# jonassibbesen/rpvg

Measured on AMD Instinct MI355X. Metric: read-pairs quantified/sec, higher is better.
Workload: dtype f64

## Files before the change

### include/rpvg_hip.h

```cpp
#ifndef RPVG_HIP_H
#define RPVG_HIP_H

#include <stdint.h>

#include "rpvg_batch.h"
#include "rpvg_rows.h"
#include "rpvg_index.h"
#include "rpvg_table.h"

#ifdef __cplusplus
extern "C" {
#endif

typedef enum rpvg_hip_status {
    RPVG_HIP_OK = 0,
    RPVG_HIP_ERR_NO_DEVICE = -1,
    RPVG_HIP_ERR_RUNTIME = -2,
    RPVG_HIP_ERR_INVALID = -3,
    RPVG_HIP_ERR_ALLOC = -4,
    RPVG_HIP_ERR_UNSUPPORTED = -5
} rpvg_hip_status;

typedef struct rpvg_hip_ctx rpvg_hip_ctx;
typedef struct rpvg_hip_batch rpvg_hip_batch;
// ... 71 lines not shown
                                double * device_matrix, uint64_t ld, double * device_counts, double * total_count);

typedef struct rpvg_hip_group_spec {
    uint32_t num_matrices;
    const uint32_t * cluster;
    const uint64_t * group_off;
    const uint64_t * group_path_off;
    const uint32_t * group_path;
    int32_t normalise;
    double collapse_precision;
} rpvg_hip_group_spec;

int rpvg_hip_groups_build(rpvg_hip_ctx * ctx, const rpvg_hip_batch * batch, const rpvg_hip_group_spec * spec,
                          rpvg_hip_groups ** groups_out);
int rpvg_hip_groups_build_from_sources(rpvg_hip_ctx * ctx, const rpvg_hip_batch * batch, uint32_t num_matrices,
                                       const uint32_t * clusters, int32_t normalise, double collapse_precision,
                                       rpvg_hip_groups ** groups_out);
int rpvg_hip_groups_build_single_paths(rpvg_hip_ctx * ctx, const rpvg_hip_batch * batch, uint32_t num_matrices,
                                       const uint32_t * clusters, int32_t normalise, double collapse_precision,
                                       rpvg_hip_groups ** groups_out);
void rpvg_hip_groups_free(rpvg_hip_ctx * ctx, rpvg_hip_groups * groups);
int rpvg_hip_groups_collapse_info(rpvg_hip_ctx * ctx, const rpvg_hip_groups * groups, uint32_t * matrices_replayed,
                                  uint32_t * rows_replaced, uint32_t * matrices_sorted_whole, uint32_t * active_rows);

int rpvg_hip_group_loglik(rpvg_hip_ctx * ctx, const rpvg_hip_groups * groups, uint32_t num_requests,
                          const uint32_t * matrix, const uint32_t * members, uint32_t width, double divisor,
                          const uint8_t * add_rowmax, double * out);

int rpvg_hip_group_conditionals(rpvg_hip_ctx * ctx, const rpvg_hip_groups * groups, uint32_t num_requests,
                                const uint32_t * matrix, const uint32_t * others, uint32_t width, double divisor,
                                double * out);

#define RPVG_HIP_FULL_MAX_SETS 0x7fffffffull
int rpvg_hip_group_full_posteriors(rpvg_hip_ctx * ctx, const rpvg_hip_groups * groups, uint32_t num_problems,
                                   const uint32_t * matrix, uint32_t group_size, const double * log_freq,
                                   double * posteriors);
uint64_t rpvg_hip_full_set_count(uint32_t columns, uint32_t group_size);

typedef struct rpvg_hip_gibbs_spec {
    uint32_t num_problems;
    uint32_t group_size;
    const uint32_t * matrix;
    const uint32_t * num_chains;
    const uint32_t * num_burn_its;
    const uint32_t * num_gibbs_its;
    const double * log_freq;
// ... 205 lines not shown
```

### rpvg_amd/csrc/row_collapse.hip

```cpp

#include "common.hpp"

#include <hipcub/hipcub.hpp>

#include <cfloat>

using namespace rpvg_hip_detail;

namespace {

constexpr int kKeyFractionBits = kCollapseKeyFractionBits;
constexpr uint32_t kMaxWindowCompares = 256;
enum : uint8_t { kRowListed = 1, kRowStoodFor = 2 };
constexpr int kCsrCellHashBits = 8;
constexpr double kEquivalentRelative = 1e-13;
constexpr uint32_t kListLdsRows = 2048;
constexpr uint32_t kSortThreads = 256;
constexpr uint32_t kBetweenThreads = 256;
constexpr uint32_t kBetweenRows = 2 * kBetweenThreads;
constexpr uint32_t kPairChunk = 256;
constexpr uint32_t kWholeMatrixBit = 0x80000000u;
constexpr uint32_t kBigListBit = 0x40000000u;
constexpr uint32_t kListSizeMask = 0x3FFFFFFFu;
constexpr uint32_t kPairwiseRows = 1024;
// ... 1134 lines not shown
        if (a.rewritten_count[m] == 0) continue;
        __syncthreads();
        adjustSearchSums(a, m, item % kAdjustSlices);
    }
}

__global__ __launch_bounds__(256) void collapseRewriteKernel(const ReplayArgs<MatrixArrays> a) {
    __shared__ uint32_t demote;
    const uint32_t num_items = a.replay_list[a.num_matrices];
    for (uint32_t item = blockIdx.x; item < num_items; item += gridDim.x) {
        const uint32_t m = a.replay_list[item];
        const uint32_t encoded = a.mat_list[m];
        __syncthreads();
        if (threadIdx.x == 0) demote = 0;
        __syncthreads();
        finishRuns(a, m, encoded & kListSizeMask, a.order + 2 * a.g.rowOffset(m), a.head_of + a.g.rowOffset(m), &demote, (encoded & kWholeMatrixBit) != 0);
    }
}

}

namespace {

constexpr uint32_t kSmallSortRows = 1024;
constexpr uint32_t kSmallSortThreads = 128;
constexpr uint32_t kSortChunkRows = 2048;
constexpr uint32_t kSortChunkThreads = 256;
constexpr uint32_t kMergeTile = 1024;
constexpr uint32_t kMergeThreads = 128;
constexpr uint32_t kSortRowBits = 20;
constexpr uint64_t kSortMaxSegmentRows = (1ull << kSortRowBits) - 1;

template <int HASH>
__device__ __forceinline__ uint64_t packSortWord(const uint64_t key, const uint32_t row) {
    constexpr int low = kCollapseLargestBits - HASH;
    const uint64_t sorted = (key & ((1ull << kCollapseMatrixShift) - 1)) >> low;
    return (sorted << (kSortRowBits + low)) | (static_cast<uint64_t>(row) << low) | (key & ((1ull << low) - 1));
}
template <int HASH>
__device__ __forceinline__ uint32_t sortWordRow(const uint64_t word) { return static_cast<uint32_t>(word >> (kCollapseLargestBits - HASH)) & ((1u << kSortRowBits) - 1); }
template <int HASH>
__device__ __forceinline__ uint64_t sortWordKey(const uint64_t word, const uint32_t matrix) {
    constexpr int low = kCollapseLargestBits - HASH;
    return (static_cast<uint64_t>(matrix) << kCollapseMatrixShift) | ((word >> (kSortRowBits + low)) << low) | (word & ((1ull << low) - 1));
}
template <int HASH>
__device__ __forceinline__ bool sortWordsSameSortedPart(const uint64_t x, const uint64_t y) {
    constexpr int shift = kSortRowBits + kCollapseLargestBits - HASH;
    return HASH ? (x >> shift) == (y >> shift) : ((x >> shift) == (y >> shift) && ((x ^ y) & ((1ull << (kCollapseLargestBits - HASH)) - 1)) == 0);
}

__device__ __forceinline__ uint64_t cellHashTerm(const uint32_t column, const double value) {
    const uint64_t cell = static_cast<uint64_t>(cellOf(value));
// ... 8 lines not shown
    return key_in[r0 + i];
}
__device__ __forceinline__ uint64_t sortKeyOfRow(const CsrArrays & g, const uint32_t p, const uint64_t r0, const uint32_t i, const uint64_t * key_in,
                                                 uint64_t * pattern_out) {
    (void) key_in;
    const CsrView mv = g.view(p);
    const double noise = mv.noise[i];
    double projection = collapseWeight(mv.G) * noise, largest = 0.0;
    uint64_t cells = cellHashTerm(mv.G, noise), pattern = 0;
    for (uint32_t e = mv.off[i]; e < mv.off[i + 1]; ++e) {
        const uint32_t c = mv.col[e];
        const double v = mv.val[e];
        projection = fma(collapseWeight(c), v, projection);
        largest = fmax(largest, v);
        cells += cellHashTerm(c, v);
        if (c < 64 && v != 0.0) pattern |= 1ull << c;
    }
    pattern_out[r0 + i] = pattern;
    constexpr int low_bits = kCollapseLargestBits - kCsrCellHashBits;
    uint64_t k = collapseSortKey(p, projection, largest);
    k = (k & ~((1ull << kCollapseLargestBits) - 1)) | (((cells * 0x9E3779B97F4A7C15ull) >> (64 - kCsrCellHashBits)) << low_bits) | (k & ((1ull << low_bits) - 1));
    return k;
}

template <typename Arrays>
struct SegmentSortArgs {
    Arrays g;
    uint32_t num_matrices;
    const uint32_t * num_matrices_dev;
    uint32_t num_items_bound;
    const uint32_t * num_items_dev;
    const uint64_t * seg_first;
    const uint32_t * item_problem;
    uint32_t segment_rows;
    uint64_t total_rows;
    const uint64_t * key_in;
    uint64_t * pattern_out;
    uint64_t * sort_key;
    uint32_t * sort_row;
    uint32_t * position_of;
    uint8_t * same_prev;
    uint32_t * stretch_start;
    uint64_t * words_a, * words_b;
    uint32_t * chunks;
    uint32_t * chunk_count;
    uint32_t chunk_capacity;
    uint32_t round;
    uint32_t rounds;
};

template <typename Arrays>
__device__ __forceinline__ void writeSortedPosition(const SegmentSortArgs<Arrays> & a, const uint32_t m, const uint64_t r0, const uint64_t position, const uint64_t word,
                                                    const uint64_t word_before, const bool has_before) {
    constexpr int HASH = Arrays::kHashBits;
    const uint32_t row = sortWordRow<HASH>(word);
    uint8_t same = 0;
    if (has_before && sortWordsSameSortedPart<HASH>(word, word_before)) {
        const typename Arrays::View mv = viewOf(m, a.g);
        const uint32_t before = sortWordRow<HASH>(word_before);
        same = (HASH ? rowsSameCells(mv, row, before) : rowsIdentical(mv, row, before)) ? 1 : 0;
    }
    a.sort_key[position] = sortWordKey<HASH>(word, m);
    a.sort_row[position] = static_cast<uint32_t>(r0 + row);
    a.position_of[r0 + row] = static_cast<uint32_t>(position);
    a.same_prev[position] = same;
    a.stretch_start[position] = same ? 0u : static_cast<uint32_t>(position);
}

template <typename Arrays>
__device__ __forceinline__ void sortChunkInLds(const SegmentSortArgs<Arrays> & a, const uint32_t m, const uint64_t r0, const uint64_t c0, const uint32_t n,
                                               const uint32_t padded, uint64_t * words) {
    constexpr int HASH = Arrays::kHashBits;
    for (uint32_t i = threadIdx.x; i < padded; i += blockDim.x) {
        words[i] = i < n ? packSortWord<HASH>(sortKeyOfRow(a.g, m, r0, static_cast<uint32_t>(c0 + i), a.key_in, a.pattern_out), static_cast<uint32_t>(c0 + i)) : ~0ull;
    }
    __syncthreads();
    for (uint32_t k = 2; k <= padded; k <<= 1) {
        for (uint32_t j = k >> 1; j > 0; j >>= 1) {
            for (uint32_t t = threadIdx.x; t < (padded >> 1); t += blockDim.x) {
                const uint32_t i = ((t & ~(j - 1)) << 1) | (t & (j - 1));
                const uint32_t l = i | j;
                const uint64_t x = words[i], y = words[l];
                if (((i & k) == 0) == (x > y)) {
                    words[i] = y;
                    words[l] = x;
                }
            }
            __syncthreads();
        }
    }
}

template <typename Arrays>
__global__ __launch_bounds__(kSmallSortThreads) void collapseSmallSortKernel(const SegmentSortArgs<Arrays> a) {
    __shared__ uint64_t words[kSmallSortRows];
    const uint32_t M = a.num_matrices_dev ? min(*a.num_matrices_dev, a.num_matrices) : a.num_matrices;
    for (uint32_t m = blockIdx.x; m < M; m += gridDim.x) {
        const uint64_t R = a.g.numRows(m);
        if (R == 0) continue;
        if (R > kSmallSortRows) {
            if (threadIdx.x == 0) {
                const uint32_t chunks = static_cast<uint32_t>((R + kSortChunkRows - 1) / kSortChunkRows);
                const uint32_t first = atomicAdd(a.chunk_count, chunks);
                for (uint32_t c = 0; c < chunks && first + c < a.chunk_capacity; ++c) {
                    a.chunks[2 * static_cast<uint64_t>(first + c)] = m;
                    a.chunks[2 * static_cast<uint64_t>(first + c) + 1] = c;
                }
            }
            continue;
        }
        const uint64_t r0 = a.g.rowOffset(m);
        const uint32_t n = static_cast<uint32_t>(R);
        uint32_t padded = 2;
        while (padded < n) padded <<= 1;
        __syncthreads();
        sortChunkInLds(a, m, r0, 0, n, padded, words);
        for (uint32_t i = threadIdx.x; i < n; i += blockDim.x) writeSortedPosition(a, m, r0, r0 + i, words[i], i ? words[i - 1] : 0ull, i != 0);
    }
}

template <typename Arrays>
__global__ __launch_bounds__(kSortChunkThreads) void collapseChunkSortKernel(const SegmentSortArgs<Arrays> a) {
    __shared__ uint64_t words[kSortChunkRows];
    const uint32_t count = min(*a.chunk_count, a.chunk_capacity);
    for (uint32_t item = blockIdx.x; item < count; item += gridDim.x) {
        const uint32_t m = a.chunks[2 * static_cast<uint64_t>(item)], chunk = a.chunks[2 * static_cast<uint64_t>(item) + 1];
        const uint64_t R = a.g.numRows(m), r0 = a.g.rowOffset(m);
        const uint64_t c0 = static_cast<uint64_t>(chunk) * kSortChunkRows;
        const uint32_t n = static_cast<uint32_t>(min(static_cast<uint64_t>(kSortChunkRows), R - c0));
        uint32_t padded = 64;
        while (padded < n) padded <<= 1;
        __syncthreads();
        sortChunkInLds(a, m, r0, c0, n, padded, words);
        for (uint32_t i = threadIdx.x; i < n; i += blockDim.x) a.words_a[r0 + c0 + i] = words[i];
    }
}

template <typename Arrays>
__global__ __launch_bounds__(kMergeThreads) void collapseMergeRoundKernel(const SegmentSortArgs<Arrays> a) {
    constexpr uint32_t kPerThread = kMergeTile / kMergeThreads;
    constexpr uint32_t kTilesPerChunk = kSortChunkRows / kMergeTile;
    const uint32_t count = min(*a.chunk_count, a.chunk_capacity) * kTilesPerChunk;
    const uint64_t * __restrict__ source = (a.round & 1) ? a.words_b : a.words_a;
    uint64_t * __restrict__ target = (a.round & 1) ? a.words_a : a.words_b;
    const uint64_t run = static_cast<uint64_t>(kSortChunkRows) << a.round;
    for (uint32_t item = blockIdx.x; item < count; item += gridDim.x) {
        const uint32_t m = a.chunks[2 * static_cast<uint64_t>(item / kTilesPerChunk)];
        const uint64_t R = a.g.numRows(m), r0 = a.g.rowOffset(m);
        const uint64_t out0 = static_cast<uint64_t>(a.chunks[2 * static_cast<uint64_t>(item / kTilesPerChunk) + 1]) * kSortChunkRows + (item % kTilesPerChunk) * kMergeTile;
        if (out0 >= R) continue;
        const uint64_t pair0 = out0 / (2 * run) * (2 * run);
        const uint64_t a1 = min(R, pair0 + run), b1 = min(R, pair0 + 2 * run);
        const uint64_t * A = source + r0 + pair0, * B = source + r0 + a1;
        const uint64_t nA = a1 - pair0, nB = b1 - a1;
        const uint64_t d = (out0 - pair0) + static_cast<uint64_t>(threadIdx.x) * kPerThread;
        if (d >= nA + nB) continue;
        uint64_t lo = d > nB ? d - nB : 0, hi = min(d, nA);
        while (lo < hi) {
            const uint64_t mid = (lo + hi) >> 1;
            if (A[mid] < B[d - mid - 1]) lo = mid + 1;
            else hi = mid;
        }
        uint64_t i = lo, j = d - lo;
        uint64_t * out = target + r0 + pair0 + d;
        const uint32_t outputs = static_cast<uint32_t>(min(static_cast<uint64_t>(kPerThread), nA + nB - d));
        uint64_t x = i < nA ? A[i] : ~0ull, y = j < nB ? B[j] : ~0ull;
        for (uint32_t k = 0; k < outputs; ++k) {
            if (x < y) {
                out[k] = x;
                ++i;
                x = i < nA ? A[i] : ~0ull;
            } else {
                out[k] = y;
                ++j;
                y = j < nB ? B[j] : ~0ull;
            }
        }
    }
}

template <typename Arrays>
__global__ __launch_bounds__(256) void collapseMergedPositionsKernel(const SegmentSortArgs<Arrays> a) {
    const uint32_t count = min(*a.chunk_count, a.chunk_capacity);
    const uint64_t * __restrict__ sorted = (a.rounds & 1) ? a.words_b : a.words_a;
    for (uint32_t item = blockIdx.x; item < count; item += gridDim.x) {
        const uint32_t m = a.chunks[2 * static_cast<uint64_t>(item)], chunk = a.chunks[2 * static_cast<uint64_t>(item) + 1];
        const uint64_t R = a.g.numRows(m), r0 = a.g.rowOffset(m);
        const uint64_t c0 = static_cast<uint64_t>(chunk) * kSortChunkRows;
        const uint32_t n = static_cast<uint32_t>(min(static_cast<uint64_t>(kSortChunkRows), R - c0));
        for (uint32_t e = threadIdx.x; e < n; e += blockDim.x) {
            const uint64_t i = c0 + e;
            writeSortedPosition(a, m, r0, r0 + i, sorted[r0 + i], i ? sorted[r0 + i - 1] : 0ull, i != 0);
        }
    }
}

template <typename Arrays>
__global__ __launch_bounds__(256) void collapseUnusedSlotsKernel(const SegmentSortArgs<Arrays> a) {
    const uint32_t M = a.num_matrices_dev ? min(*a.num_matrices_dev, a.num_matrices) : a.num_matrices;
    const uint32_t items = a.num_items_dev ? min(*a.num_items_dev, a.num_items_bound) : a.num_items_bound;
    const uint64_t unused = collapseSortKey(a.num_matrices, 0.0, 0.0);
    auto fill = [&](const uint64_t r) {
        a.sort_key[r] = unused;
        a.sort_row[r] = static_cast<uint32_t>(r);
        a.position_of[r] = static_cast<uint32_t>(r);
        a.same_prev[r] = 0;
        a.stretch_start[r] = static_cast<uint32_t>(r);
        a.pattern_out[r] = 0;
    };
    for (uint32_t item = blockIdx.x; item < items; item += gridDim.x) {
// ... 36 lines not shown
    DeviceBuffer<uint32_t> row_out, order, head, pair_column, marked_list, pairs, between_items, row_items, list_index;
    DeviceBuffer<uint32_t> stretch;
    DeviceBuffer<uint64_t> pair_base;
    DeviceBuffer<uint8_t> pair_table;
    DeviceBuffer<double> pair_bound;
    DeviceBuffer<uint8_t> bytes;
    DeviceBuffer<unsigned char> sort_tmp;
    DeviceBuffer<uint64_t> csr_key, csr_pattern;
    DeviceBuffer<uint32_t> csr_row, csr_segments;
    DeviceBuffer<uint64_t> words_a, words_b;
    DeviceBuffer<uint32_t> chunks, chunk_count;
};

struct SegmentSortPlan {
    const uint32_t * num_matrices_dev = nullptr;
    uint32_t num_items_bound = 0;
    const uint32_t * num_items_dev = nullptr;
    const uint64_t * seg_first = nullptr;
    const uint32_t * item_problem = nullptr;
    uint32_t segment_rows = 0;
    uint64_t * pattern_out = nullptr;
    uint64_t max_segment_rows = 0;
};

template <typename Arrays>
hipError_t queueCollapseStages(const Arrays & arrays, const uint32_t M, const uint64_t total_rows, const double precision, const uint64_t * key,
                               const uint32_t * row, const uint32_t * segment_begin, const uint32_t * segment_end, const bool segmented, DeviceBuffer<uint32_t> & info, double * rowmax, uint32_t * mat_fast,
                               uint32_t * mat_mid, CollapseTemporaries * tmp, hipStream_t st, const SegmentSortPlan * plan = nullptr, hipEvent_t sorted = nullptr,
                               std::function<hipError_t(hipStream_t, const SearchParts *)> * held_back_runs = nullptr) {
    hipError_t e = hipSuccess;
    auto ok = [&](hipError_t r) { if (e == hipSuccess) e = r; return e == hipSuccess; };
    const uint64_t mark_words = (total_rows + 31) / 32;
    const uint64_t num_words = 2 + 2 * static_cast<uint64_t>(M) + 1 + mark_words + 5;
    const uint32_t pair_capacity = static_cast<uint32_t>(std::min<uint64_t>(4 * total_rows + 4096, 0x20000000ull));
    if (tmp->key_out.count != total_rows) ok(tmp->key_out.alloc(total_rows));
    if (tmp->row_out.count != total_rows) ok(tmp->row_out.alloc(total_rows));
    const uint64_t active_words = (total_rows + 3) / 4;
    ok(info.alloc(kInfoWords + num_words + active_words + M));
    ok(tmp->order.alloc(2 * total_rows));
    ok(tmp->head.alloc(total_rows));
    ok(tmp->pair_column.alloc(total_rows));
    ok(tmp->pair_bound.alloc(2 * total_rows));
    ok(tmp->pair_pattern.alloc(total_rows));
    ok(tmp->marked_list.alloc(total_rows));
    ok(tmp->pairs.alloc(2 * static_cast<size_t>(pair_capacity)));
    ok(tmp->between_items.alloc(2 * (total_rows / kBetweenRows + M)));
// ... 3 lines not shown
    ok(tmp->pair_table.alloc(kPairTableBytes));
    ok(tmp->bytes.alloc(3 * total_rows));
    ok(tmp->stretch.alloc(4 * total_rows));
    int matrix_bits = 1;
    while ((1u << matrix_bits) < M + 1) ++matrix_bits;
    const int begin_bit = kCollapseLargestBits - Arrays::kHashBits, end_bit = segmented ? kCollapseMatrixShift : kCollapseMatrixShift + matrix_bits;
    size_t sort_bytes = 0;
    auto sort = [&](void * scratch) {
        return segmented ? hipcub::DeviceSegmentedRadixSort::SortPairs(scratch, sort_bytes, key, tmp->key_out.ptr, row,
                                                                       tmp->row_out.ptr, static_cast<int>(total_rows), static_cast<int>(M),
                                                                       segment_begin, segment_end, begin_bit, end_bit, st)
                         : hipcub::DeviceRadixSort::SortPairs(scratch, sort_bytes, key, tmp->key_out.ptr, row,
                                                              tmp->row_out.ptr, static_cast<int>(total_rows), begin_bit, end_bit, st);
    };
    if (e == hipSuccess && !plan) ok(sort(nullptr));
    uint32_t * stretch_start = tmp->stretch.ptr, * stretch_first = stretch_start + total_rows, * stretch_end = stretch_first + total_rows,
             * position_of = stretch_end + total_rows;
    size_t scan_bytes = 0;
    auto scan = [&](void * scratch) {
        return hipcub::DeviceScan::InclusiveScan(scratch, scan_bytes, stretch_start, stretch_first, hipcub::Max(), static_cast<int>(total_rows), st);
    };
    if (e == hipSuccess) ok(scan(nullptr));
    ok(tmp->sort_tmp.alloc(std::max(sort_bytes, scan_bytes)));
    uint32_t chunk_capacity = 0, merge_rounds = 0;
    if (plan) {
        chunk_capacity = static_cast<uint32_t>(std::min<uint64_t>(total_rows / kSortChunkRows + M + 1, 0x7fffffffull));
        const uint64_t max_chunks = (plan->max_segment_rows + kSortChunkRows - 1) / kSortChunkRows;
        while ((1ull << merge_rounds) < max_chunks) ++merge_rounds;
        ok(tmp->words_a.alloc(total_rows));
        ok(tmp->words_b.alloc(total_rows));
        ok(tmp->chunks.alloc(2 * static_cast<size_t>(chunk_capacity)));
        ok(tmp->chunk_count.alloc(1));
    }
    if (e != hipSuccess) return e;
    uint32_t * pair_bytes = info.ptr + kInfoWords, * mat_flag = pair_bytes + 2, * replay_list = mat_flag + M, * marked_bits = replay_list + M + 1,
             * marked_count = marked_bits + mark_words, * pair_counts = marked_count + 1, * between_count = pair_counts + 2,
             * row_item_count = between_count + 1, * mat_list = pair_bytes + num_words + active_words;
    uint8_t * same_prev = tmp->bytes.ptr, * close = same_prev + total_rows, * barrier = close + total_rows;
    uint8_t * active = reinterpret_cast<uint8_t *>(pair_bytes + num_words);
    ok(zeroAsync(info.ptr, (kInfoWords + num_words + active_words) * sizeof(uint32_t), st));
    if (!plan) ok(sort(tmp->sort_tmp.ptr));
    PairScanArgs<Arrays> a;
    a.total_rows = total_rows;
    a.precision = precision;
    a.sort_key = tmp->key_out.ptr;
    a.sort_row = tmp->row_out.ptr;
    a.g = arrays;
    a.same_prev = same_prev;
    a.stretch_first = stretch_start;
    a.stretch_end = stretch_end;
    a.position_of = position_of;
// ... 15 lines not shown
        SegmentSortArgs<Arrays> c;
        c.g = arrays;
        c.num_matrices = M;
        c.num_matrices_dev = plan->num_matrices_dev;
        c.num_items_bound = plan->num_items_bound;
        c.num_items_dev = plan->num_items_dev;
        c.seg_first = plan->seg_first;
        c.item_problem = plan->item_problem;
        c.segment_rows = plan->segment_rows;
        c.total_rows = total_rows;
        c.key_in = key;
        c.pattern_out = plan->pattern_out;
        c.sort_key = tmp->key_out.ptr;
        c.sort_row = tmp->row_out.ptr;
        c.position_of = position_of;
        c.same_prev = same_prev;
        c.stretch_start = stretch_start;
        c.words_a = tmp->words_a.ptr;
        c.words_b = tmp->words_b.ptr;
        c.chunks = tmp->chunks.ptr;
        c.chunk_count = tmp->chunk_count.ptr;
        c.chunk_capacity = chunk_capacity;
        c.round = 0;
        c.rounds = merge_rounds;
        if (Arrays::kHashBits) {
            collapseUnusedSlotsKernel<Arrays><<<dim3(std::max<uint32_t>(1, std::min<uint32_t>(plan->num_items_bound, 8 * small_grid))), dim3(256), 0, st>>>(c);
        }
        collapseSmallSortKernel<Arrays><<<dim3(std::max<uint32_t>(1, std::min<uint32_t>(M, 16 * small_grid))), dim3(kSmallSortThreads), 0, st>>>(c);
        if (plan->max_segment_rows > kSmallSortRows) {
            collapseChunkSortKernel<Arrays><<<dim3(4 * small_grid), dim3(kSortChunkThreads), 0, st>>>(c);
            for (uint32_t round = 0; round < merge_rounds; ++round) {
                c.round = round;
                collapseMergeRoundKernel<Arrays><<<dim3(8 * small_grid), dim3(kMergeThreads), 0, st>>>(c);
            }
            collapseMergedPositionsKernel<Arrays><<<dim3(4 * small_grid), dim3(256), 0, st>>>(c);
        }
    } else {
        collapseSamePrevKernel<Arrays><<<dim3(row_blocks), dim3(256), 0, st>>>(a);
    }
    if (sorted) ok(hipEventRecord(sorted, st));
    ok(scan(tmp->sort_tmp.ptr));
    a.stretch_first = stretch_first;
    collapseStretchEndKernel<Arrays><<<dim3(row_blocks), dim3(256), 0, st>>>(a);
    collapseForwardPairsKernel<Arrays><<<dim3(row_blocks), dim3(256), 0, st>>>(a);
    collapseMarkPairsKernel<Arrays><<<dim3(small_grid), dim3(64), 0, st>>>(a);
    a.pair_count = pair_counts + 1;
    collapseAroundPairsKernel<Arrays><<<dim3(256), dim3(64), 0, st>>>(a);
    collapseActivePairsKernel<Arrays><<<dim3(small_grid), dim3(64), 0, st>>>(a);
    ReplayArgs<Arrays> r;
    r.num_matrices = M;
    r.precision = precision;
    r.g = arrays;
    r.mat_flag = mat_flag;
    r.active = active;
    r.sort_row = tmp->row_out.ptr;
    r.position_of = position_of;
    r.stretch_end = stretch_end;
    r.rowmax = rowmax;
    r.mat_fast = mat_fast;
// ... 205 lines not shown
    ok(hipGetLastError());
    if (e != hipSuccess) return e;
    return queueCollapseStages(arrays, P, total_rows, precision, tmp->csr_key.ptr, tmp->csr_row.ptr, segment_begin, segment_end, segmented, work.info, nullptr,
                               nullptr, nullptr, tmp.get(), st, nullptr, sorted);
}

extern "C" int rpvg_hip_groups_collapse_info(rpvg_hip_ctx * ctx, const rpvg_hip_groups * groups, uint32_t * matrices_replayed,
                                             uint32_t * rows_replaced, uint32_t * matrices_sorted_whole, uint32_t * active_rows) {
    RPVG_REQUIRE(ctx && groups, "rpvg_hip_groups_collapse_info: NULL argument");
    uint32_t info[kInfoWords] = {0};
    if (groups->collapse_info.ptr) {
        std::lock_guard<std::mutex> lock(ctx->mutex);
        RPVG_HIP_CHECK(hipSetDevice(ctx->device));
        RPVG_HIP_CHECK(groups->waitCollapse(ctx->stream));
        RPVG_HIP_CHECK(hipMemcpyAsync(info, groups->collapse_info.ptr, sizeof(info), hipMemcpyDeviceToHost, ctx->stream));
        RPVG_HIP_CHECK(hipStreamSynchronize(ctx->stream));
    }
    if (matrices_replayed) *matrices_replayed = info[kInfoMatrices];
    if (rows_replaced) *rows_replaced = info[kInfoRowsReplaced];
    if (matrices_sorted_whole) *matrices_sorted_whole = info[kInfoWholeMatrices];
    if (active_rows) *active_rows = info[kInfoActiveRows];
    return RPVG_HIP_OK;
}
```

### rpvg_amd/hip.py

```python
from __future__ import annotations

import ctypes as C
import os
from typing import List, Optional, Sequence, Tuple

import numpy as np

from .batch import CClusterBatch, ClusterBatch

_HERE = os.path.dirname(os.path.abspath(__file__))
LIB_PATH = os.path.join(_HERE, "csrc", "librpvg_hip.so")

EXPORTS = [
    "rpvg_hip_device_count", "rpvg_hip_create", "rpvg_hip_create_uploader", "rpvg_hip_destroy", "rpvg_hip_last_error", "rpvg_hip_synchronize",
    "rpvg_hip_device_info", "rpvg_hip_malloc", "rpvg_hip_free", "rpvg_hip_memcpy_h2d", "rpvg_hip_memcpy_d2h",
    "rpvg_hip_batch_upload", "rpvg_hip_batch_free", "rpvg_hip_em_solve", "rpvg_hip_em_dense",
    "rpvg_hip_dense_from_cluster", "rpvg_hip_groups_build", "rpvg_hip_groups_free", "rpvg_hip_groups_collapse_info", "rpvg_hip_group_loglik",
    "rpvg_hip_synth_dense_cluster", "rpvg_hip_stats_get", "rpvg_hip_stats_reset", "rpvg_hip_stats_intervals", "rpvg_hip_em_kernel_name",
    "rpvg_hip_gibbs_read_counts", "rpvg_hip_min_path_cover", "rpvg_hip_min_path_cover_any", "rpvg_hip_cover_limits", "rpvg_hip_bounded_pair_posteriors", "rpvg_hip_pair_posteriors_get", "rpvg_hip_pair_posteriors_free",
    "rpvg_hip_em_dense_sharded", "rpvg_hip_synth_dense_rows", "rpvg_hip_synth_dense_cluster_batch", "rpvg_hip_comm_unique_id", "rpvg_hip_comm_init",
    "rpvg_hip_comm_destroy", "rpvg_hip_comm_allreduce_sum_f64", "rpvg_hip_comm_init_all", "rpvg_hip_gather", "rpvg_hip_host_register", "rpvg_hip_host_unregister", "rpvg_hip_group_conditionals",
    "rpvg_hip_group_gibbs", "rpvg_hip_group_gibbs_polyploid", "rpvg_hip_gibbs_sets_get", "rpvg_hip_gibbs_sets_free",
    "rpvg_hip_alignments_upload", "rpvg_hip_alignments_free", "rpvg_hip_read_rows_build", "rpvg_hip_read_rows_to_batch",
    "rpvg_hip_read_rows_view", "rpvg_hip_read_rows_sizes", "rpvg_hip_read_rows_free", "rpvg_hip_path_clusters", "rpvg_hip_debug_log",
    "rpvg_hip_nested_subset_em", "rpvg_hip_subset_em_get", "rpvg_hip_subset_em_free",
    "rpvg_hip_batch_cluster_totals", "rpvg_hip_batch_has_source_columns", "rpvg_hip_batch_source_columns_sizes",
    "rpvg_hip_batch_source_columns_get", "rpvg_hip_groups_build_from_sources", "rpvg_hip_groups_build_single_paths", "rpvg_hip_batch_upload_begin", "rpvg_hip_batch_upload_finish", "rpvg_hip_create_with_streams",
    "rpvg_hip_batch_upload_finish_queue", "rpvg_hip_batch_upload_finish_wait",
    "rpvg_hip_batch_upload_segments", "rpvg_hip_pinned_alloc", "rpvg_hip_pinned_free", "rpvg_hip_thread_wait_spin_us",
    "rpvg_hip_group_full_posteriors", "rpvg_hip_full_set_count",
    "rpvg_hip_frag_length_fit", "rpvg_hip_frag_length_table", "rpvg_hip_frag_length_table_get", "rpvg_hip_frag_length_table_free",
    "rpvg_hip_effective_lengths", "rpvg_hip_alignments_set_effective_lengths", "rpvg_hip_frag_length_eval",
    "rpvg_hip_align_index_create", "rpvg_hip_align_index_free", "rpvg_hip_align_index_add", "rpvg_hip_align_index_finish",
    "rpvg_hip_align_index_frag_counts", "rpvg_hip_align_index_view", "rpvg_hip_align_index_alignments",
    "rpvg_hip_path_table_upload", "rpvg_hip_path_table_free", "rpvg_hip_read_rows_to_batch_with_paths", "rpvg_hip_batch_path_group_ids",
    "rpvg_hip_name_groups_limits", "rpvg_hip_align_index_name_groups", "rpvg_hip_name_groups_view", "rpvg_hip_name_groups_free",
    "rpvg_hip_estimates_table_build", "rpvg_hip_estimates_table_tpm", "rpvg_hip_estimates_table_view", "rpvg_hip_estimates_table_limits",
    "rpvg_hip_estimates_table_free",
    "rpvg_hip_align_index_alignments_collapsed",
    "rpvg_hip_batch_rows_sizes", "rpvg_hip_batch_rows_get",
]

COMM_ID_BYTES = 128


class EngineError(RuntimeError):
    pass


class CEmProblems(C.Structure):
    _fields_ = [("num_problems", C.c_uint32), ("cluster", C.c_void_p), ("col_off", C.c_void_p), ("col_path", C.c_void_p),
                ("collapse_precision", C.c_double)]


class CEmResults(C.Structure):
    _fields_ = [("abundances", C.c_void_p), ("noise_count", C.c_void_p), ("total_count", C.c_void_p),
                ("iterations", C.c_void_p)]


class CGroupSpec(C.Structure):
    _fields_ = [("num_matrices", C.c_uint32), ("cluster", C.c_void_p), ("group_off", C.c_void_p),
                ("group_path_off", C.c_void_p), ("group_path", C.c_void_p), ("normalise", C.c_int32),
                ("collapse_precision", C.c_double)]
# ... 625 lines not shown
        _check(lib().rpvg_hip_gibbs_read_counts(self.handle, batch.handle, C.byref(probs), C.c_void_p(init.ctypes.data),
                                                C.c_void_p(init_noise.ctypes.data), C.c_void_p(n.ctypes.data), C.c_void_p(sd.ctypes.data),
                                                C.c_uint32(thin), C.c_double(gamma), C.c_void_p(noise.ctypes.data),
                                                C.c_void_p(abund.ctypes.data)), "rpvg_hip_gibbs_read_counts")
        out, at_n, at_a = [], 0, 0
        for p in range(P):
            k, w = int(n[p]), int(widths[p])
            out.append((noise[at_n:at_n + k], abund[at_a:at_a + k * w].reshape(k, w)))
            at_n, at_a = at_n + k, at_a + k * w
        return out

    def min_path_cover(self, batch: DeviceBatch, clusters: Sequence[int], extra: Optional[Sequence[int]] = None) -> List[List[int]]:
        cl = np.ascontiguousarray(clusters, dtype=np.uint32)
        n_paths = [int(batch.host.cluster_path_off[k + 1] - batch.host.cluster_path_off[k]) for k in clusters]
        off = np.zeros(len(cl) + 1, dtype=np.uint64)
        off[1:] = np.cumsum(n_paths if extra is None else [n + int(x) for n, x in zip(n_paths, extra)])
        cover = np.zeros(int(off[-1]), dtype=np.uint32)
        size = np.zeros(len(cl), dtype=np.uint32)
        _check(lib().rpvg_hip_min_path_cover(self.handle, batch.handle, C.c_uint32(len(cl)), C.c_void_p(cl.ctypes.data),
                                             C.c_void_p(off.ctypes.data), C.c_void_p(cover.ctypes.data),
                                             C.c_void_p(size.ctypes.data)), "rpvg_hip_min_path_cover")
        return [[int(x) for x in cover[int(off[i]):int(off[i]) + int(size[i])]] for i in range(len(cl))]

    def min_path_cover_any(self, batch: DeviceBatch, clusters: Sequence[int], extra: Optional[Sequence[int]] = None, grid_min_work: int = 0,
                           order: bool = False):
        cl = np.ascontiguousarray(clusters, dtype=np.uint32)
        n_paths = [int(batch.host.cluster_path_off[k + 1] - batch.host.cluster_path_off[k]) for k in clusters]
        off = np.zeros(len(cl) + 1, dtype=np.uint64)
        off[1:] = np.cumsum(n_paths if extra is None else [n + int(x) for n, x in zip(n_paths, extra)])
        cover = np.zeros(int(off[-1]), dtype=np.uint32)
        chosen = np.zeros(int(off[-1]), dtype=np.uint32)
        size = np.zeros(len(cl), dtype=np.uint32)
        _check(lib().rpvg_hip_min_path_cover_any(self.handle, batch.handle, C.c_uint32(len(cl)), C.c_void_p(cl.ctypes.data),
                                                 C.c_void_p(off.ctypes.data), C.c_void_p(cover.ctypes.data), C.c_void_p(size.ctypes.data),
                                                 C.c_uint64(grid_min_work), C.c_void_p(chosen.ctypes.data if order else None)),
               "rpvg_hip_min_path_cover_any")
        covers = [[int(x) for x in cover[int(off[i]):int(off[i]) + int(size[i])]] for i in range(len(cl))]
        if not order:
            return covers
        orders = [None if n_paths[i] and int(chosen[int(off[i])]) == 0xFFFFFFFF else [int(x) for x in chosen[int(off[i]):int(off[i]) + int(size[i])]]
                  for i in range(len(cl))]
        return covers, orders

    def malloc(self, nbytes: int) -> int:
        p = C.c_void_p()
        _check(lib().rpvg_hip_malloc(self.handle, C.c_uint64(nbytes), C.byref(p)), "rpvg_hip_malloc")
# ... 146 lines not shown
```

Baseline: 2.394 billion.

## Replace LDS bitonic segment sort with register and wave-shuffle bitonic sort

```diff
diff --git a/include/rpvg_hip.h b/include/rpvg_hip.h
--- a/include/rpvg_hip.h
+++ b/include/rpvg_hip.h
@@ -117,6 +117,8 @@
 void rpvg_hip_groups_free(rpvg_hip_ctx * ctx, rpvg_hip_groups * groups);
 int rpvg_hip_groups_collapse_info(rpvg_hip_ctx * ctx, const rpvg_hip_groups * groups, uint32_t * matrices_replayed,
                                   uint32_t * rows_replaced, uint32_t * matrices_sorted_whole, uint32_t * active_rows);
+int rpvg_hip_segment_sort_words(rpvg_hip_ctx * ctx, const uint64_t * words, const uint64_t * segment_off, uint32_t num_segments,
+                                uint64_t * out);
 
 int rpvg_hip_group_loglik(rpvg_hip_ctx * ctx, const rpvg_hip_groups * groups, uint32_t num_requests,
                           const uint32_t * matrix, const uint32_t * members, uint32_t width, double divisor,
diff --git a/rpvg_amd/csrc/row_collapse.hip b/rpvg_amd/csrc/row_collapse.hip
--- a/rpvg_amd/csrc/row_collapse.hip
+++ b/rpvg_amd/csrc/row_collapse.hip
@@ -1,5 +1,6 @@
 
 #include "common.hpp"
+#include "segment_sort_plan.hpp"
 
 #include <hipcub/hipcub.hpp>
 
@@ -1180,13 +1181,14 @@
 
 namespace {
 
-constexpr uint32_t kSmallSortRows = 1024;
-constexpr uint32_t kSmallSortThreads = 128;
-constexpr uint32_t kSortChunkRows = 2048;
-constexpr uint32_t kSortChunkThreads = 256;
+constexpr uint32_t kSmallSortRows = rpvg_sort::kSmallSortRows;
+constexpr uint32_t kOneWaveSortRows = rpvg_sort::kOneWaveRows;
+constexpr uint32_t kSmallSortThreads = rpvg_sort::kSmallSortWaves * rpvg_sort::kWaveLanes;
+constexpr uint32_t kSortChunkRows = rpvg_sort::kChunkRows;
+constexpr uint32_t kSortChunkThreads = rpvg_sort::kChunkWaves * rpvg_sort::kWaveLanes;
 constexpr uint32_t kMergeTile = 1024;
 constexpr uint32_t kMergeThreads = 128;
-constexpr uint32_t kSortRowBits = 20;
+constexpr uint32_t kSortRowBits = rpvg_sort::kRowBits;
 constexpr uint64_t kSortMaxSegmentRows = (1ull << kSortRowBits) - 1;
 
 template <int HASH>
@@ -1241,6 +1243,14 @@
     k = (k & ~((1ull << kCollapseLargestBits) - 1)) | (((cells * 0x9E3779B97F4A7C15ull) >> (64 - kCsrCellHashBits)) << low_bits) | (k & ((1ull << low_bits) - 1));
     return k;
 }
+
+struct WordArrays {
+    const uint64_t * words;
+    const uint64_t * segment_off;
+    uint64_t * out;
+    __device__ __forceinline__ uint64_t rowOffset(const uint32_t s) const { return segment_off[s]; }
+    __device__ __forceinline__ uint64_t numRows(const uint32_t s) const { return segment_off[s + 1] - segment_off[s]; }
+};
 
 template <typename Arrays>
 struct SegmentSortArgs {
@@ -1265,8 +1275,13 @@
     uint32_t * chunk_count;
     uint32_t chunk_capacity;
     uint32_t round;
-    uint32_t rounds;
 };
+
+template <typename Arrays>
+__device__ __forceinline__ uint64_t sortWordOfRow(const SegmentSortArgs<Arrays> & a, const uint32_t m, const uint64_t r0, const uint32_t i) {
+    return packSortWord<Arrays::kHashBits>(sortKeyOfRow(a.g, m, r0, i, a.key_in, a.pattern_out), i);
+}
+__device__ __forceinline__ uint64_t sortWordOfRow(const SegmentSortArgs<WordArrays> & a, const uint32_t, const uint64_t r0, const uint32_t i) { return a.g.words[r0 + i]; }
 
 template <typename Arrays>
 __device__ __forceinline__ void writeSortedPosition(const SegmentSortArgs<Arrays> & a, const uint32_t m, const uint64_t r0, const uint64_t position, const uint64_t word,
@@ -1285,56 +1300,195 @@
     a.same_prev[position] = same;
     a.stretch_start[position] = same ? 0u : static_cast<uint32_t>(position);
 }
-
-template <typename Arrays>
-__device__ __forceinline__ void sortChunkInLds(const SegmentSortArgs<Arrays> & a, const uint32_t m, const uint64_t r0, const uint64_t c0, const uint32_t n,
-                                               const uint32_t padded, uint64_t * words) {
-    constexpr int HASH = Arrays::kHashBits;
-    for (uint32_t i = threadIdx.x; i < padded; i += blockDim.x) {
-        words[i] = i < n ? packSortWord<HASH>(sortKeyOfRow(a.g, m, r0, static_cast<uint32_t>(c0 + i), a.key_in, a.pattern_out), static_cast<uint32_t>(c0 + i)) : ~0ull;
-    }
+__device__ __forceinline__ void writeSortedPosition(const SegmentSortArgs<WordArrays> & a, const uint32_t, const uint64_t, const uint64_t position, const uint64_t word,
+                                                    const uint64_t, const bool) {
+    a.g.out[position] = word;
+}
+
+template <uint32_t D>
+__device__ __forceinline__ uint64_t wordOfLaneXor(const uint64_t x) {
+    static_assert(D == 1 || D == 2 || D == 4 || D == 8, "lane distance");
+    const int lo = static_cast<int>(static_cast<uint32_t>(x)), hi = static_cast<int>(static_cast<uint32_t>(x >> 32));
+    int other_lo, other_hi;
+    if constexpr (D == 1) {
+        other_lo = __builtin_amdgcn_update_dpp(0, lo, 0xB1, 0xF, 0xF, true);
+        other_hi = __builtin_amdgcn_update_dpp(0, hi, 0xB1, 0xF, 0xF, true);
+    } else if constexpr (D == 2) {
+        other_lo = __builtin_amdgcn_update_dpp(0, lo, 0x4E, 0xF, 0xF, true);
+        other_hi = __builtin_amdgcn_update_dpp(0, hi, 0x4E, 0xF, 0xF, true);
+    } else {
+        constexpr int pattern = static_cast<int>((D << 10) | 0x1F);
+        other_lo = __builtin_amdgcn_ds_swizzle(lo, pattern);
+        other_hi = __builtin_amdgcn_ds_swizzle(hi, pattern);
+    }
+    return (static_cast<uint64_t>(static_cast<uint32_t>(other_hi)) << 32) | static_cast<uint32_t>(other_lo);
+}
+
+template <int E, uint32_t D>
+__device__ __forceinline__ void exchangeStage(uint64_t (&v)[E], const bool keep_smaller) {
+#pragma unroll
+    for (int e = 0; e < E; ++e) {
+        if constexpr (D == 16 || D == 32) {
+            const uint32_t lo = static_cast<uint32_t>(v[e]), hi = static_cast<uint32_t>(v[e] >> 32);
+            const auto l = D == 16 ? __builtin_amdgcn_permlane16_swap(lo, lo, false, false) : __builtin_amdgcn_permlane32_swap(lo, lo, false, false);
+            const auto h = D == 16 ? __builtin_amdgcn_permlane16_swap(hi, hi, false, false) : __builtin_amdgcn_permlane32_swap(hi, hi, false, false);
+            const uint64_t lower = (static_cast<uint64_t>(h[0]) << 32) | l[0], upper = (static_cast<uint64_t>(h[1]) << 32) | l[1];
+            v[e] = ((lower < upper) == keep_smaller) ? lower : upper;
+        } else {
+            const uint64_t other = wordOfLaneXor<D>(v[e]);
+            v[e] = ((other < v[e]) == keep_smaller) ? other : v[e];
+        }
+    }
+}
+
+template <int E, int WAVES>
+__device__ __forceinline__ void exchangeThroughLds(uint64_t (&v)[E], uint64_t * lds, const uint32_t t, const uint32_t distance, const bool keep_smaller) {
+    constexpr uint32_t T = rpvg_sort::kWaveLanes * WAVES;
+#pragma unroll
+    for (int e = 0; e < E; ++e) lds[e * T + t] = v[e];
     __syncthreads();
-    for (uint32_t k = 2; k <= padded; k <<= 1) {
-        for (uint32_t j = k >> 1; j > 0; j >>= 1) {
-            for (uint32_t t = threadIdx.x; t < (padded >> 1); t += blockDim.x) {
-                const uint32_t i = ((t & ~(j - 1)) << 1) | (t & (j - 1));
-                const uint32_t l = i | j;
-                const uint64_t x = words[i], y = words[l];
-                if (((i & k) == 0) == (x > y)) {
-                    words[i] = y;
-                    words[l] = x;
+#pragma unroll
+    for (int e = 0; e < E; ++e) {
+        const uint64_t other = lds[e * T + (t ^ distance)];
+        v[e] = ((other < v[e]) == keep_smaller) ? other : v[e];
+    }
+    __syncthreads();
+}
+
+template <int E>
+__device__ __forceinline__ void inLaneStage(uint64_t (&v)[E], const uint32_t t, const uint32_t k, const uint32_t j) {
+#pragma unroll
+    for (uint32_t e = 0; e < static_cast<uint32_t>(E); ++e) {
+        if (e & j) continue;
+        const bool ascending = rpvg_sort::ascendingAt(t * E + e, k);
+        const uint64_t x = v[e], y = v[e | j];
+        const bool swap = (x > y) == ascending;
+        v[e] = swap ? y : x;
+        v[e | j] = swap ? x : y;
+    }
+}
+
+template <int E>
+__device__ __forceinline__ void inLaneStageDirected(uint64_t (&v)[E], const bool ascending, const uint32_t j) {
+#pragma unroll
+    for (uint32_t e = 0; e < static_cast<uint32_t>(E); ++e) {
+        if (e & j) continue;
+        const uint64_t x = v[e], y = v[e | j];
+        const bool swap = (x > y) == ascending;
+        v[e] = swap ? y : x;
+        v[e | j] = swap ? x : y;
+    }
+}
+
+template <int E, int WAVES>
+__device__ __forceinline__ void sortWordsInRegisters(uint64_t (&v)[E], uint64_t * lds, const uint32_t t) {
+    constexpr uint32_t N = rpvg_sort::kWaveLanes * WAVES * E;
+    (void) lds;
+#pragma unroll
+    for (uint32_t k = 2; k <= static_cast<uint32_t>(E); k <<= 1) {
+#pragma unroll
+        for (uint32_t j = k >> 1; j > 0; j >>= 1) inLaneStage<E>(v, t, k, j);
+    }
+#pragma unroll 1
+    for (uint32_t k = 2 * E; k <= N; k <<= 1) {
+        const bool ascending = rpvg_sort::ascendingAt(t * E, k);
+#pragma unroll 1
+        for (uint32_t j = k >> 1; j >= static_cast<uint32_t>(E); j >>= 1) {
+            const uint32_t distance = rpvg_sort::laneDistance(j, E);
+            const bool keep_smaller = ((t & distance) == 0) == ascending;
+            if (rpvg_sort::stageKind(j, E) == rpvg_sort::kAcrossWaves) {
+                if constexpr (WAVES > 1) exchangeThroughLds<E, WAVES>(v, lds, t, distance, keep_smaller);
+            } else {
+                switch (distance) {
+                    case 1: exchangeStage<E, 1>(v, keep_smaller); break;
+                    case 2: exchangeStage<E, 2>(v, keep_smaller); break;
+                    case 4: exchangeStage<E, 4>(v, keep_smaller); break;
+                    case 8: exchangeStage<E, 8>(v, keep_smaller); break;
+                    case 16: exchangeStage<E, 16>(v, keep_smaller); break;
+                    default: exchangeStage<E, 32>(v, keep_smaller); break;
                 }
             }
-            __syncthreads();
-        }
-    }
-}
-
-template <typename Arrays>
-__global__ __launch_bounds__(kSmallSortThreads) void collapseSmallSortKernel(const SegmentSortArgs<Arrays> a) {
+        }
+#pragma unroll
+        for (uint32_t j = static_cast<uint32_t>(E) >> 1; j > 0; j >>= 1) inLaneStageDirected<E>(v, ascending, j);
+    }
+}
+
+template <int WAVES>
+__device__ __forceinline__ void sortGroupSync() {
+    if constexpr (WAVES > 1) {
+        __syncthreads();
+    } else {
+        __builtin_amdgcn_fence(__ATOMIC_ACQ_REL, "wavefront");
+        __builtin_amdgcn_wave_barrier();
+    }
+}
+
+template <typename Arrays, int E, int WAVES>
+__device__ __forceinline__ void sortSegmentWords(const SegmentSortArgs<Arrays> & a, const uint32_t m, const uint64_t r0, const uint64_t c0, const uint32_t n,
+                                                 uint64_t * image, const uint32_t t) {
+    constexpr uint32_t T = rpvg_sort::kWaveLanes * WAVES;
+    uint64_t v[E];
+#pragma unroll
+    for (int e = 0; e < E; ++e) {
+        const uint32_t i = e * T + t;
+        v[e] = i < n ? sortWordOfRow(a, m, r0, static_cast<uint32_t>(c0 + i)) : rpvg_sort::kPaddingWord;
+    }
+    sortWordsInRegisters<E, WAVES>(v, image, t);
+#pragma unroll
+    for (int e = 0; e < E; ++e) image[t * E + e] = v[e];
+    sortGroupSync<WAVES>();
+}
+
+template <typename Arrays, int WAVES>
+__device__ __forceinline__ void sortSegmentOfGroup(const SegmentSortArgs<Arrays> & a, const uint32_t m, const uint64_t r0, const uint64_t c0, const uint32_t n,
+                                                   uint64_t * image, const uint32_t t) {
+    switch (rpvg_sort::classOfGroup(n, WAVES).words_per_lane) {
+        case 1: sortSegmentWords<Arrays, 1, WAVES>(a, m, r0, c0, n, image, t); break;
+        case 2: sortSegmentWords<Arrays, 2, WAVES>(a, m, r0, c0, n, image, t); break;
+        case 4: sortSegmentWords<Arrays, 4, WAVES>(a, m, r0, c0, n, image, t); break;
+        default: sortSegmentWords<Arrays, 8, WAVES>(a, m, r0, c0, n, image, t); break;
+    }
+}
+
+template <typename Arrays>
+__global__ __launch_bounds__(kSmallSortThreads) __attribute__((amdgpu_waves_per_eu(4))) void collapseSmallSortKernel(const SegmentSortArgs<Arrays> a) {
     __shared__ uint64_t words[kSmallSortRows];
     const uint32_t M = a.num_matrices_dev ? min(*a.num_matrices_dev, a.num_matrices) : a.num_matrices;
-    for (uint32_t m = blockIdx.x; m < M; m += gridDim.x) {
-        const uint64_t R = a.g.numRows(m);
-        if (R == 0) continue;
-        if (R > kSmallSortRows) {
-            if (threadIdx.x == 0) {
-                const uint32_t chunks = static_cast<uint32_t>((R + kSortChunkRows - 1) / kSortChunkRows);
-                const uint32_t first = atomicAdd(a.chunk_count, chunks);
-                for (uint32_t c = 0; c < chunks && first + c < a.chunk_capacity; ++c) {
-                    a.chunks[2 * static_cast<uint64_t>(first + c)] = m;
-                    a.chunks[2 * static_cast<uint64_t>(first + c) + 1] = c;
+    const uint32_t wave = __builtin_amdgcn_readfirstlane(threadIdx.x / rpvg_sort::kWaveLanes), lane = threadIdx.x % rpvg_sort::kWaveLanes;
+    for (uint64_t m0 = static_cast<uint64_t>(blockIdx.x) * rpvg_sort::kSmallSortWaves; m0 < M; m0 += static_cast<uint64_t>(gridDim.x) * rpvg_sort::kSmallSortWaves) {
+        if (m0 + wave < M) {
+            const uint32_t m = static_cast<uint32_t>(m0 + wave);
+            const uint64_t R = a.g.numRows(m);
+            if (R > kSmallSortRows) {
+                if (lane == 0) {
+                    const uint32_t chunks = static_cast<uint32_t>((R + kSortChunkRows - 1) / kSortChunkRows);
+                    const uint32_t first = atomicAdd(a.chunk_count, chunks);
+                    for (uint32_t c = 0; c < chunks && first + c < a.chunk_capacity; ++c) {
+                        a.chunks[2 * static_cast<uint64_t>(first + c)] = m;
+                        a.chunks[2 * static_cast<uint64_t>(first + c) + 1] = c;
+                    }
                 }
-            }
-            continue;
-        }
-        const uint64_t r0 = a.g.rowOffset(m);
-        const uint32_t n = static_cast<uint32_t>(R);
-        uint32_t padded = 2;
-        while (padded < n) padded <<= 1;
-        __syncthreads();
-        sortChunkInLds(a, m, r0, 0, n, padded, words);
-        for (uint32_t i = threadIdx.x; i < n; i += blockDim.x) writeSortedPosition(a, m, r0, r0 + i, words[i], i ? words[i - 1] : 0ull, i != 0);
+            } else if (R > 0 && R <= kOneWaveSortRows) {
+                const uint64_t r0 = a.g.rowOffset(m);
+                const uint32_t n = static_cast<uint32_t>(R);
+                uint64_t * image = words + wave * kOneWaveSortRows;
+                sortSegmentOfGroup<Arrays, 1>(a, m, r0, 0, n, image, lane);
+                for (uint32_t i = lane; i < n; i += rpvg_sort::kWaveLanes) writeSortedPosition(a, m, r0, r0 + i, image[i], i ? image[i - 1] : 0ull, i != 0);
+                sortGroupSync<1>();
+            }
+        }
+        for (uint32_t w = 0; w < rpvg_sort::kSmallSortWaves && m0 + w < M; ++w) {
+            const uint32_t m = static_cast<uint32_t>(m0 + w);
+            const uint64_t R = a.g.numRows(m);
+            if (R <= kOneWaveSortRows || R > kSmallSortRows) continue;
+            const uint64_t r0 = a.g.rowOffset(m);
+            const uint32_t n = static_cast<uint32_t>(R);
+            __syncthreads();
+            sortSegmentWords<Arrays, rpvg_sort::kMaxWordsPerLane, rpvg_sort::kSmallSortWaves>(a, m, r0, 0, n, words, threadIdx.x);
+            for (uint32_t i = threadIdx.x; i < n; i += blockDim.x) writeSortedPosition(a, m, r0, r0 + i, words[i], i ? words[i - 1] : 0ull, i != 0);
+            __syncthreads();
+        }
     }
 }
 
@@ -1347,10 +1501,8 @@
         const uint64_t R = a.g.numRows(m), r0 = a.g.rowOffset(m);
         const uint64_t c0 = static_cast<uint64_t>(chunk) * kSortChunkRows;
         const uint32_t n = static_cast<uint32_t>(min(static_cast<uint64_t>(kSortChunkRows), R - c0));
-        uint32_t padded = 64;
-        while (padded < n) padded <<= 1;
-        __syncthreads();
-        sortChunkInLds(a, m, r0, c0, n, padded, words);
+        __syncthreads();
+        sortSegmentOfGroup<Arrays, rpvg_sort::kChunkWaves>(a, m, r0, c0, n, words, threadIdx.x);
         for (uint32_t i = threadIdx.x; i < n; i += blockDim.x) a.words_a[r0 + c0 + i] = words[i];
     }
 }
@@ -1360,12 +1512,14 @@
     constexpr uint32_t kPerThread = kMergeTile / kMergeThreads;
     constexpr uint32_t kTilesPerChunk = kSortChunkRows / kMergeTile;
     const uint32_t count = min(*a.chunk_count, a.chunk_capacity) * kTilesPerChunk;
-    const uint64_t * __restrict__ source = (a.round & 1) ? a.words_b : a.words_a;
-    uint64_t * __restrict__ target = (a.round & 1) ? a.words_a : a.words_b;
-    const uint64_t run = static_cast<uint64_t>(kSortChunkRows) << a.round;
+    const uint64_t * __restrict__ source = rpvg_sort::sourceBuffer(a.round) ? a.words_b : a.words_a;
+    uint64_t * __restrict__ target = rpvg_sort::targetBuffer(a.round) ? a.words_b : a.words_a;
+    const uint64_t run = rpvg_sort::runLength(a.round);
     for (uint32_t item = blockIdx.x; item < count; item += gridDim.x) {
         const uint32_t m = a.chunks[2 * static_cast<uint64_t>(item / kTilesPerChunk)];
-        const uint64_t R = a.g.numRows(m), r0 = a.g.rowOffset(m);
+        const uint64_t R = a.g.numRows(m);
+        if (!rpvg_sort::roundHasWork(R, a.round)) continue;
+        const uint64_t r0 = a.g.rowOffset(m);
         const uint64_t out0 = static_cast<uint64_t>(a.chunks[2 * static_cast<uint64_t>(item / kTilesPerChunk) + 1]) * kSortChunkRows + (item % kTilesPerChunk) * kMergeTile;
         if (out0 >= R) continue;
         const uint64_t pair0 = out0 / (2 * run) * (2 * run);
@@ -1401,10 +1555,10 @@
 template <typename Arrays>
 __global__ __launch_bounds__(256) void collapseMergedPositionsKernel(const SegmentSortArgs<Arrays> a) {
     const uint32_t count = min(*a.chunk_count, a.chunk_capacity);
-    const uint64_t * __restrict__ sorted = (a.rounds & 1) ? a.words_b : a.words_a;
     for (uint32_t item = blockIdx.x; item < count; item += gridDim.x) {
         const uint32_t m = a.chunks[2 * static_cast<uint64_t>(item)], chunk = a.chunks[2 * static_cast<uint64_t>(item) + 1];
         const uint64_t R = a.g.numRows(m), r0 = a.g.rowOffset(m);
+        const uint64_t * __restrict__ sorted = rpvg_sort::finalBuffer(R) ? a.words_b : a.words_a;
         const uint64_t c0 = static_cast<uint64_t>(chunk) * kSortChunkRows;
         const uint32_t n = static_cast<uint32_t>(min(static_cast<uint64_t>(kSortChunkRows), R - c0));
         for (uint32_t e = threadIdx.x; e < n; e += blockDim.x) {
@@ -1487,6 +1641,23 @@
     uint64_t * pattern_out = nullptr;
     uint64_t max_segment_rows = 0;
 };
+
+inline uint32_t segmentSortChunkCapacity(const uint64_t total_rows, const uint32_t M) {
+    return static_cast<uint32_t>(std::min<uint64_t>(total_rows / kSortChunkRows + M + 1, 0x7fffffffull));
+}
+template <typename Arrays>
+void launchSegmentSort(SegmentSortArgs<Arrays> c, const uint32_t M, const uint64_t max_segment_rows, const uint32_t small_grid, hipStream_t st) {
+    const uint32_t pairs = (M + rpvg_sort::kSmallSortWaves - 1) / rpvg_sort::kSmallSortWaves;
+    collapseSmallSortKernel<Arrays><<<dim3(std::max<uint32_t>(1, std::min<uint32_t>(pairs, 16 * small_grid))), dim3(kSmallSortThreads), 0, st>>>(c);
+    if (max_segment_rows <= kSmallSortRows) return;
+    collapseChunkSortKernel<Arrays><<<dim3(4 * small_grid), dim3(kSortChunkThreads), 0, st>>>(c);
+    const uint32_t merge_rounds = rpvg_sort::mergeRoundsOf(max_segment_rows);
+    for (uint32_t round = 0; round < merge_rounds; ++round) {
+        c.round = round;
+        collapseMergeRoundKernel<Arrays><<<dim3(8 * small_grid), dim3(kMergeThreads), 0, st>>>(c);
+    }
+    collapseMergedPositionsKernel<Arrays><<<dim3(4 * small_grid), dim3(256), 0, st>>>(c);
+}
 
 template <typename Arrays>
 hipError_t queueCollapseStages(const Arrays & arrays, const uint32_t M, const uint64_t total_rows, const double precision, const uint64_t * key,
@@ -1536,11 +1707,9 @@
     };
     if (e == hipSuccess) ok(scan(nullptr));
     ok(tmp->sort_tmp.alloc(std::max(sort_bytes, scan_bytes)));
-    uint32_t chunk_capacity = 0, merge_rounds = 0;
+    uint32_t chunk_capacity = 0;
     if (plan) {
-        chunk_capacity = static_cast<uint32_t>(std::min<uint64_t>(total_rows / kSortChunkRows + M + 1, 0x7fffffffull));
-        const uint64_t max_chunks = (plan->max_segment_rows + kSortChunkRows - 1) / kSortChunkRows;
-        while ((1ull << merge_rounds) < max_chunks) ++merge_rounds;
+        chunk_capacity = segmentSortChunkCapacity(total_rows, M);
         ok(tmp->words_a.alloc(total_rows));
         ok(tmp->words_b.alloc(total_rows));
         ok(tmp->chunks.alloc(2 * static_cast<size_t>(chunk_capacity)));
@@ -1602,19 +1771,10 @@
         c.chunk_count = tmp->chunk_count.ptr;
         c.chunk_capacity = chunk_capacity;
         c.round = 0;
-        c.rounds = merge_rounds;
         if (Arrays::kHashBits) {
             collapseUnusedSlotsKernel<Arrays><<<dim3(std::max<uint32_t>(1, std::min<uint32_t>(plan->num_items_bound, 8 * small_grid))), dim3(256), 0, st>>>(c);
         }
-        collapseSmallSortKernel<Arrays><<<dim3(std::max<uint32_t>(1, std::min<uint32_t>(M, 16 * small_grid))), dim3(kSmallSortThreads), 0, st>>>(c);
-        if (plan->max_segment_rows > kSmallSortRows) {
-            collapseChunkSortKernel<Arrays><<<dim3(4 * small_grid), dim3(kSortChunkThreads), 0, st>>>(c);
-            for (uint32_t round = 0; round < merge_rounds; ++round) {
-                c.round = round;
-                collapseMergeRoundKernel<Arrays><<<dim3(8 * small_grid), dim3(kMergeThreads), 0, st>>>(c);
-            }
-            collapseMergedPositionsKernel<Arrays><<<dim3(4 * small_grid), dim3(256), 0, st>>>(c);
-        }
+        launchSegmentSort(c, M, plan->max_segment_rows, small_grid, st);
     } else {
         collapseSamePrevKernel<Arrays><<<dim3(row_blocks), dim3(256), 0, st>>>(a);
     }
@@ -1866,3 +2026,47 @@
     if (active_rows) *active_rows = info[kInfoActiveRows];
     return RPVG_HIP_OK;
 }
+
+extern "C" int rpvg_hip_segment_sort_words(rpvg_hip_ctx * ctx, const uint64_t * words, const uint64_t * segment_off, uint32_t num_segments, uint64_t * out) {
+    RPVG_REQUIRE(ctx && segment_off, "rpvg_hip_segment_sort_words: NULL argument");
+    if (num_segments == 0) return RPVG_HIP_OK;
+    uint64_t longest = 0;
+    for (uint32_t s = 0; s < num_segments; ++s) {
+        RPVG_REQUIRE(segment_off[s] <= segment_off[s + 1], "rpvg_hip_segment_sort_words: segment_off descends at segment %u", s);
+        longest = std::max(longest, segment_off[s + 1] - segment_off[s]);
+    }
+    const uint64_t total = segment_off[num_segments];
+    RPVG_REQUIRE(segment_off[0] == 0 && total <= 0x7fffffffull, "rpvg_hip_segment_sort_words: segment_off must start at 0 and end below 2^31");
+    if (total == 0) return RPVG_HIP_OK;
+    RPVG_REQUIRE(words && out, "rpvg_hip_segment_sort_words: NULL argument");
+    std::lock_guard<std::mutex> lock(ctx->mutex);
+    RPVG_HIP_CHECK(hipSetDevice(ctx->device));
+    hipStream_t st = ctx->stream;
+    DeviceBuffer<uint64_t> d_words, d_off, d_out, words_a, words_b;
+    DeviceBuffer<uint32_t> chunks, chunk_count;
+    const uint32_t chunk_capacity = segmentSortChunkCapacity(total, num_segments);
+    RPVG_HIP_CHECK(d_words.upload(words, total, st));
+    RPVG_HIP_CHECK(d_off.upload(segment_off, static_cast<size_t>(num_segments) + 1, st));
+    RPVG_HIP_CHECK(d_out.alloc(total));
+    RPVG_HIP_CHECK(words_a.alloc(total));
+    RPVG_HIP_CHECK(words_b.alloc(total));
+    RPVG_HIP_CHECK(chunks.alloc(2 * static_cast<size_t>(chunk_capacity)));
+    RPVG_HIP_CHECK(chunk_count.alloc(1));
+    RPVG_HIP_CHECK(zeroAsync(chunk_count.ptr, sizeof(uint32_t), st));
+    SegmentSortArgs<WordArrays> c{};
+    c.g.words = d_words.ptr;
+    c.g.segment_off = d_off.ptr;
+    c.g.out = d_out.ptr;
+    c.num_matrices = num_segments;
+    c.total_rows = total;
+    c.words_a = words_a.ptr;
+    c.words_b = words_b.ptr;
+    c.chunks = chunks.ptr;
+    c.chunk_count = chunk_count.ptr;
+    c.chunk_capacity = chunk_capacity;
+    launchSegmentSort(c, num_segments, longest, 256, st);
+    RPVG_HIP_CHECK(hipGetLastError());
+    RPVG_HIP_CHECK(d_out.download(out, st));
+    RPVG_HIP_CHECK(hipStreamSynchronize(st));
+    return RPVG_HIP_OK;
+}
diff --git a/rpvg_amd/csrc/segment_sort_plan.hpp b/rpvg_amd/csrc/segment_sort_plan.hpp
--- /dev/null
+++ b/rpvg_amd/csrc/segment_sort_plan.hpp
@@ -0,0 +1,66 @@
+#ifndef RPVG_SEGMENT_SORT_PLAN_HPP
+#define RPVG_SEGMENT_SORT_PLAN_HPP
+
+#include <cstdint>
+
+#if defined(__HIPCC__)
+#define RPVG_SORT_FN __host__ __device__ inline
+#else
+#define RPVG_SORT_FN inline
+#endif
+
+namespace rpvg_sort {
+
+constexpr uint32_t kWaveLanes = 64;
+constexpr uint32_t kMaxWordsPerLane = 8;
+constexpr uint32_t kOneWaveRows = kWaveLanes * kMaxWordsPerLane;
+constexpr uint32_t kSmallSortWaves = 2;
+constexpr uint32_t kSmallSortRows = kSmallSortWaves * kOneWaveRows;
+constexpr uint32_t kChunkWaves = 4;
+constexpr uint32_t kChunkRows = kChunkWaves * kWaveLanes * kMaxWordsPerLane;
+constexpr uint32_t kRowBits = 20;
+constexpr uint64_t kMaxSegmentRows = (1ull << kRowBits) - 1;
+constexpr uint64_t kPaddingWord = ~0ull;
+
+struct SizeClass {
+    uint32_t padded, words_per_lane, waves;
+};
+RPVG_SORT_FN bool operator==(const SizeClass & x, const SizeClass & y) {
+    return x.padded == y.padded && x.words_per_lane == y.words_per_lane && x.waves == y.waves;
+}
+
+RPVG_SORT_FN SizeClass classOfGroup(const uint32_t rows, const uint32_t waves) {
+    uint32_t E = 1;
+    while (E < kMaxWordsPerLane && rows > waves * kWaveLanes * E) E <<= 1;
+    return SizeClass{waves * kWaveLanes * E, E, waves};
+}
+RPVG_SORT_FN SizeClass smallClassOf(const uint32_t rows) {
+    return rows <= kOneWaveRows ? classOfGroup(rows, 1) : SizeClass{kSmallSortRows, kMaxWordsPerLane, kSmallSortWaves};
+}
+RPVG_SORT_FN SizeClass chunkClassOf(const uint32_t rows) { return classOfGroup(rows, kChunkWaves); }
+
+enum StageKind { kInLane = 0, kInWave = 1, kAcrossWaves = 2 };
+RPVG_SORT_FN StageKind stageKind(const uint32_t j, const uint32_t words_per_lane) {
+    return j < words_per_lane ? kInLane : j < kWaveLanes * words_per_lane ? kInWave : kAcrossWaves;
+}
+RPVG_SORT_FN uint32_t partnerOf(const uint32_t i, const uint32_t j) { return i ^ j; }
+RPVG_SORT_FN bool ascendingAt(const uint32_t i, const uint32_t k) { return (i & k) == 0; }
+RPVG_SORT_FN bool keepsSmaller(const uint32_t i, const uint32_t k, const uint32_t j) { return ((i & j) == 0) == ascendingAt(i, k); }
+RPVG_SORT_FN uint32_t laneDistance(const uint32_t j, const uint32_t words_per_lane) { return j / words_per_lane; }
+
+RPVG_SORT_FN uint32_t chunksOf(const uint64_t rows) { return static_cast<uint32_t>((rows + kChunkRows - 1) / kChunkRows); }
+RPVG_SORT_FN uint32_t mergeRoundsOf(const uint64_t rows) {
+    const uint64_t chunks = (rows + kChunkRows - 1) / kChunkRows;
+    uint32_t rounds = 0;
+    while ((1ull << rounds) < chunks) ++rounds;
+    return rounds;
+}
+RPVG_SORT_FN uint64_t runLength(const uint32_t round) { return static_cast<uint64_t>(kChunkRows) << round; }
+RPVG_SORT_FN bool roundHasWork(const uint64_t rows, const uint32_t round) { return round < mergeRoundsOf(rows); }
+RPVG_SORT_FN uint32_t sourceBuffer(const uint32_t round) { return round & 1; }
+RPVG_SORT_FN uint32_t targetBuffer(const uint32_t round) { return (round + 1) & 1; }
+RPVG_SORT_FN uint32_t finalBuffer(const uint64_t rows) { return mergeRoundsOf(rows) & 1; }
+
+}
+
+#endif
diff --git a/rpvg_amd/hip.py b/rpvg_amd/hip.py
--- a/rpvg_amd/hip.py
+++ b/rpvg_amd/hip.py
@@ -39,6 +39,7 @@
     "rpvg_hip_estimates_table_free",
     "rpvg_hip_align_index_alignments_collapsed",
     "rpvg_hip_batch_rows_sizes", "rpvg_hip_batch_rows_get",
+    "rpvg_hip_segment_sort_words",
 ]
 
 COMM_ID_BYTES = 128
@@ -710,6 +711,15 @@
                                              C.c_void_p(size.ctypes.data)), "rpvg_hip_min_path_cover")
         return [[int(x) for x in cover[int(off[i]):int(off[i]) + int(size[i])]] for i in range(len(cl))]
 
+    def segment_sort_words(self, words, segment_off) -> np.ndarray:
+        w = np.ascontiguousarray(words, dtype=np.uint64)
+        off = np.ascontiguousarray(segment_off, dtype=np.uint64)
+        assert len(off) >= 1 and int(off[-1]) == len(w)
+        out = np.zeros(len(w), dtype=np.uint64)
+        _check(lib().rpvg_hip_segment_sort_words(self.handle, C.c_void_p(w.ctypes.data), C.c_void_p(off.ctypes.data),
+                                                 C.c_uint32(len(off) - 1), C.c_void_p(out.ctypes.data)), "rpvg_hip_segment_sort_words")
+        return out
+
     def min_path_cover_any(self, batch: DeviceBatch, clusters: Sequence[int], extra: Optional[Sequence[int]] = None, grid_min_work: int = 0,
                            order: bool = False):
         cl = np.ascontiguousarray(clusters, dtype=np.uint32)
```

Measured after the change: 2.427 billion, median of 6. 1.4% higher.
